# Schaudge/cellranger

Measured on AMD Instinct MI355X. Metric: M reads/sec barcode-correct+UMI-count, higher is better.
Workload: dtype u32/u64 integer keys; f64 posterior

## Files before the change

cellranger_amd/_lib.py:

```python
import ctypes as C
import os

import numpy as np

PKG = os.path.dirname(os.path.abspath(__file__))
LIB_PATH = os.environ.get("CRGPU_LIB_PATH") or os.path.join(PKG, "libcrgpu.so")

MISS = 0xFFFFFFFF
NO_FEATURE = 0xFFFFFFFF
MAX_LIB = 16
FLAG_LIB_MASK = 0x0F
FLAG_CB_HAS_N = 0x10
FLAG_NONTXOMIC = 0x20

COUNTS_VALID, COUNTS_CORRECTED, COUNTS_PRIOR = 0, 1, 2
T_NAMES = ["pack", "match", "correct", "keys", "sort_scatter", "dedup", "matrix", "synth", "sort_hist", "scan", "comm", "feature"]
UNIQUE_ID_BYTES = 128
OPT_BUFFERS_UNCHANGED_BETWEEN_CALLS = 0
STAT_SORT_REFINISHED = 1
STAT_RL_COUNTS_FROM_FINISH = 15


class CrgpuError(RuntimeError):
    def __init__(self, code, msg):
        super().__init__("crgpu error %d: %s" % (code, msg))
        self.code = code


class Records(C.Structure):
    _fields_ = [
        ("n", C.c_uint64),
        ("umi_len", C.c_uint32),
        ("d_bc_idx", C.c_void_p),
        ("d_umi", C.c_void_p),
        ("d_umi_qualn", C.c_void_p),
        ("d_feature", C.c_void_p),
        ("d_flags", C.c_void_p),
        ("d_umi_len", C.c_void_p),
        ("d_probe_idx", C.c_void_p),
    ]


class MatrixView(C.Structure):
# ... 330 lines not shown
```

cellranger_amd/csrc/common.h:

```cpp
#pragma once

#include <hip/hip_runtime.h>

#include <cstdarg>
#include <cstdint>
#include <cstdio>
#include <cstring>
#include <map>
#include <mutex>
#include <set>
#include <string>
#include <vector>

#include "../../include/crgpu.h"

#define CR_WAVE 64
#define CR_SCALAR_N_WITHOUT_FLAGS 40

struct WlTables {
    bool set = false;
    uint32_t n = 0;
    uint32_t bitsA = 0;
    uint32_t bitsB = 0;
    uint32_t *d_offA = nullptr;
// ... 115 lines not shown

    bool canon_set = false;
    uint32_t n_canon = 0, cb_len = 0;
    std::vector<uint32_t> canon_sorted;
    std::vector<uint32_t> canon_order;

    uint32_t n_segments = 0;
    uint32_t seg_n[CRGPU_MAX_SEGMENTS] = {0}, seg_len[CRGPU_MAX_SEGMENTS] = {0};
    std::vector<uint32_t> seg_seq[CRGPU_MAX_SEGMENTS];

    WlTables wl[CRGPU_MAX_LIB];
    FeaturePattern pat[CRGPU_MAX_LIB];
    FeatureExtractorSet fx[CRGPU_MAX_LIB];
    FxPendingSet fxp;
    uint32_t *d_canon_keys = nullptr;
    unsigned long long *d_hot_image = nullptr;
#define CR_REC_SETS 4
    MissRecords recs[CR_REC_SETS];
    uint32_t rec_next = 0;
    KeyHistograms ghist;
    std::map<const void *, size_t> lds_attr_done;
    uint32_t n_xcc = 0;
    uint64_t last_distinct_keys = 0, last_low_support_candidates = 0;
    uint64_t rl_counts_from_finish = 0;
    uint64_t sort_refinished = 0;
    uint64_t k1_split_rounds = 0;
    uint64_t feature_resumed_reads = 0;
    uint64_t feature_fast_launches = 0;
    uint64_t feature_reads_requeued = 0;
    uint64_t comm_bytes[3] = {0, 0, 0};
    uint64_t sort_fallbacks = 0;
    uint64_t probe_segments[3] = {0, 0, 0};
    uint32_t probe_seg_cap = 0xFFFFFFFFu;
    uint32_t ordmag_batch = 0;
    uint32_t ed_lds_features = 0xFFFFFFFFu;
    uint32_t ss_wave_min = 64, ss_wg_min = 4096, ss_task_batch = 0;

    double max_expected_errors = 1.7976931348623157e308;
    double confidence_threshold = 0.975;
    double *d_ptab = nullptr;

    KeyLayout layout;
    DenseIndex dense;
    uint8_t *d_on_target = nullptr;
    uint32_t n_target_features = 0;
    uint64_t target_min_reads = 0;
// ... 136 lines not shown
```

cellranger_amd/csrc/ctx.hip:

```cpp
#include <cmath>

#include <cstdio>
#include <cstdlib>

#include "common.h"

static thread_local std::string g_thread_err;

void cr_set_thread_error(const char *msg) { g_thread_err = msg; }

int cr_fail(crgpu_ctx *ctx, int code, const char *fmt, ...) {
    char buf[1024];
    va_list ap;
    va_start(ap, fmt);
    vsnprintf(buf, sizeof(buf), fmt, ap);
    va_end(ap);
    if (ctx)
        ctx->err = buf;
    else
        g_thread_err = buf;
    return code;
}

extern "C" int crgpu_abi_version(void) { return CRGPU_ABI_VERSION; }
// ... 246 lines not shown
        case CRGPU_STAT_COMM_BYTES_C1:
        case CRGPU_STAT_COMM_BYTES_C2:
        case CRGPU_STAT_COMM_BYTES_C3:
            *value_out = ctx->comm_bytes[which - CRGPU_STAT_COMM_BYTES_C1];
            return CRGPU_OK;
        case CRGPU_STAT_FEATURE_RESUMED_READS:
            *value_out = ctx->feature_resumed_reads;
            return CRGPU_OK;
        case CRGPU_STAT_FEATURE_FAST_LAUNCHES:
            *value_out = ctx->feature_fast_launches;
            return CRGPU_OK;
        case CRGPU_STAT_MISS_RECORD_SETS: {
            uint64_t k = 0;
            for (const MissRecords &r : ctx->recs) k += r.valid ? 1u : 0u;
            *value_out = k;
            return CRGPU_OK;
        }
        case CRGPU_STAT_DISTINCT_KEYS:
            *value_out = ctx->last_distinct_keys;
            return CRGPU_OK;
        case CRGPU_STAT_LOW_SUPPORT_CANDIDATES:
            *value_out = ctx->last_low_support_candidates;
            return CRGPU_OK;
        case CRGPU_STAT_FEATURE_READS_REQUEUED:
            *value_out = ctx->feature_reads_requeued;
            return CRGPU_OK;
        case CRGPU_STAT_PROBE_SEGMENTS_WAVE:
        case CRGPU_STAT_PROBE_SEGMENTS_WORKGROUP:
        case CRGPU_STAT_PROBE_SEGMENTS_GLOBAL:
            *value_out = ctx->probe_segments[which - CRGPU_STAT_PROBE_SEGMENTS_WAVE];
            return CRGPU_OK;
        default:
            return cr_fail(ctx, CRGPU_EINVAL, "crgpu_get_stat: unknown counter %d", which);
    }
}

void cr_invalidate(crgpu_ctx *ctx) {
    cr_drop_miss_records(ctx);
    cr_drop_feature_pending(ctx);
    ctx->ghist.valid = false;
}
void cr_invalidate_range(crgpu_ctx *ctx, const void *p, uint64_t bytes) {
    if (!p || !bytes) return;
    const uintptr_t a = (uintptr_t)p, b = a + bytes;
    auto hits = [&](const void *q, uint64_t len) { return q && (uintptr_t)q < b && (uintptr_t)q + len > a; };
    for (MissRecords &r : ctx->recs)
// ... 302 lines not shown
```

cellranger_amd/csrc/dedup.hip:

```cpp
#include "block_utils.h"
#include "common.h"

int cr_scan_small(crgpu_ctx *ctx, uint32_t *d_data, uint64_t n, uint32_t *d_total_out);
int cr_partition_by_owner(crgpu_ctx *ctx, const uint64_t *d_in, uint64_t *d_out, uint64_t n, uint32_t sh_bc,
                          uint32_t n_ranks, const uint32_t *bounds, uint64_t *counts_out);

#define NONE32 0xFFFFFFFFu

struct crgpu_counts {
    uint64_t n_triplets = 0, n_molecules = 0;
    uint32_t *d_bc = nullptr, *d_feature = nullptr, *d_count = nullptr;
    uint64_t *d_mkeys = nullptr;
    uint32_t *d_mreads = nullptr;
    uint32_t *d_corr_reads = nullptr;
    uint32_t *d_filt_reads = nullptr;
    int32_t *d_mprobe = nullptr;
    uint32_t *d_back = nullptr;
    uint32_t n_back = 0;
    uint32_t n_canon = 0;
    KeyLayout layout;
    bool pt_valid = false;
    uint32_t pt_n_probes = 0;
    uint64_t n_pt = 0;
    uint32_t *d_pt_bc = nullptr, *d_pt_probe = nullptr, *d_pt_count = nullptr;
// ... 1621 lines not shown
            rl_heads.valid = false;
        }
    }
    const uint64_t *keys = keys_rw;
    const uint32_t *vals = vals_rw;
    uint32_t nd32 = 0;
    {
        CrTimer t(ctx, CRGPU_T_DEDUP, n_keys);
        CR_TRY(run_lengths(ctx, keys, 1u, n_keys, ukey, upos, d_block, d_total, rl_heads.valid));
    }
    CR_TRY(read_u32(ctx, d_total, &nd32));
    const uint64_t nd = nd32;

    const uint64_t st_bytes = ((nd + 1) & ~1ull) * sizeof(uint16_t) + 4;
    DevBuf corr_b, incall_b, st_b, minidx_b;
    CR_TRY(dmalloc(ctx, minidx_b, nd * sizeof(uint32_t)));
    CR_TRY(dmalloc(ctx, corr_b, nd * sizeof(uint32_t)));
    CR_TRY(dmalloc(ctx, incall_b, nd * sizeof(uint32_t)));
    CR_TRY(dmalloc(ctx, st_b, st_bytes));
    uint32_t *corr = corr_b.as<uint32_t>(), *inc_all = incall_b.as<uint32_t>(), *minidx = minidx_b.as<uint32_t>();
    uint16_t *st = st_b.as<uint16_t>();
    const bool overlap = CrFork::enabled(ctx, nd);
    CrFork fork(ctx);
    DevBuf heads_b, giant_b, best_b;
    if (overlap) CR_TRY(fork.mark());
    {
        const bool timing_was = ctx->timing;
        if (overlap) ctx->timing = false;
        struct TimingBack {
            crgpu_ctx *c;
            bool v;
            ~TimingBack() { c->timing = v; }
        } timing_back{ctx, timing_was};
        CrTimer t(ctx, CRGPU_T_DEDUP);
        CR_HIP(ctx, hipMemsetAsync(inc_all, 0, nd * sizeof(uint32_t), ctx->stream));
        CR_HIP(ctx, hipMemsetAsync(st, 0, st_bytes, ctx->stream));
        CR_HIP(ctx, hipMemsetAsync(minidx, 0xFF, nd * sizeof(uint32_t), ctx->stream));
        const uint64_t n_tiles = (nd + UC_TILE - 1) / UC_TILE;
        CR_TRY(dmalloc(ctx, heads_b, 2 * n_tiles * sizeof(uint32_t)));
        uint32_t *tile_first = heads_b.as<uint32_t>(), *tile_last = tile_first + n_tiles;
#ifndef UC_GRID_WG
#define UC_GRID_WG 5u
#endif
        hipLaunchKernelGGL(k_correct_umis_tiled, dim3(cr_grid(n_tiles, 1, 256u * UC_GRID_WG)), dim3(256), 0, ctx->stream, kl, ukey,
                           upos, nd, n_keys, tile_first, tile_last, corr, st, inc_all, minidx);
        if (n_tiles > 1) {
            const size_t lds_small = (2 * UES_CAP + UES_BUCKETS * 8) * sizeof(uint32_t);
            const size_t lds_large = (2 * UE_CAP + UE_BUCKETS * 8) * sizeof(uint32_t);
            cr_allow_lds(ctx, (const void *)k_correct_umis_edges<false>, lds_large);
            cr_allow_lds(ctx, (const void *)k_giant_probe, lds_large);
            const uint64_t max_items = nd / (UE_CAP / 2) + 16;
            CR_TRY(dmalloc(ctx, giant_b, max_items * sizeof(GiantItem) + 16));
            CR_TRY(dmalloc(ctx, best_b, nd * sizeof(unsigned long long)));
            uint32_t *n_giant = reinterpret_cast<uint32_t *>(giant_b.as<unsigned char>());
            GiantItem *items = reinterpret_cast<GiantItem *>(giant_b.as<unsigned char>() + 16);
            unsigned long long *best = best_b.as<unsigned long long>();
            CR_HIP(ctx, hipMemsetAsync(n_giant, 0, sizeof(uint32_t), ctx->stream));
            hipLaunchKernelGGL(k_correct_umis_edges<true>, dim3(cr_grid(n_tiles - 1, 1, 256u * 6u)), dim3(UES_THREADS), lds_small,
                               ctx->stream, kl, ukey, upos, nd, n_keys, tile_first, tile_last, corr, st, inc_all, minidx, items, n_giant);
            hipLaunchKernelGGL(k_correct_umis_edges<false>, dim3(cr_grid(n_tiles - 1, 1, 256u * 2u)), dim3(UE_THREADS),
                               lds_large, ctx->stream, kl, ukey, upos, nd, n_keys, tile_first, tile_last, corr, st, inc_all,
                               minidx, items, n_giant);
            hipLaunchKernelGGL(k_giant_init, dim3(512), dim3(UE_THREADS), 0, ctx->stream, kl, ukey, upos, nd, n_keys, items,
                               n_giant, best);
            hipLaunchKernelGGL(k_giant_probe, dim3(512), dim3(UE_THREADS), lds_large, ctx->stream, kl, ukey, upos, nd, n_keys,
                               items, n_giant, best);
            hipLaunchKernelGGL(k_giant_final, dim3(512), dim3(UE_THREADS), 0, ctx->stream, upos, nd, n_keys, items, n_giant, best,
                               corr, st, inc_all, minidx);
        }
        CR_HIP(ctx, hipGetLastError());
    }

    {
        DevBuf cand_b, h_b, v_b;
        CR_TRY(dmalloc(ctx, cand_b, nd));
        CR_TRY(dmalloc(ctx, h_b, nd * sizeof(uint32_t)));
        CR_TRY(dmalloc(ctx, v_b, nd * sizeof(uint32_t)));
        const uint32_t vbits = cr_ceil_log2(nd ? nd : 1);
        uint32_t n_cand32 = 0;
        if (overlap) CR_TRY(fork.side(fork.t0));
        {
            CrTimer t(ctx, CRGPU_T_DEDUP);
            const uint64_t n_ftiles = (nd + LF_TILE - 1) / LF_TILE;
            hipLaunchKernelGGL(k_group_candidates, dim3(cr_grid(n_ftiles, 1, 256u * 2u)), dim3(LF_THREADS), 0, ctx->stream, kl, ukey, nd,
                               cand_b.as<uint8_t>());
// ... 92 lines not shown
        uint64_t tile;
        const uint32_t nb = cp_blocks(nd, &tile);
        const MolFlagTargeted flag_t{st, ukey, upos, inc_all, n_keys, nd, tf};
        const MolFlag flag_p{st};
        if (tf.min_reads)
            hipLaunchKernelGGL(k_mt_count<MolFlagTargeted>, dim3(nb), dim3(CP_BLOCK), 0, ctx->stream, flag_t, ukey, L.sh_feat(), nd,
                               tile, d_block, d_heads);
        else
            hipLaunchKernelGGL(k_mt_count<MolFlag>, dim3(nb), dim3(CP_BLOCK), 0, ctx->stream, flag_p, ukey, L.sh_feat(), nd, tile,
                               d_block, d_heads);
        CR_TRY(cr_scan_small(ctx, d_block, nb, d_total));
        CR_TRY(cr_scan_small(ctx, d_heads, nb, d_total_h));
        if (tf.min_reads)
            hipLaunchKernelGGL(k_mt_write<MolFlagTargeted>, dim3(nb), dim3(CP_BLOCK), 0, ctx->stream, flag_t, emit, L.sh_bc(),
                               L.sh_feat(), L.bits_feat, nd, tile, d_block, d_heads, res->d_bc, res->d_feature, tpos_b.as<uint32_t>(),
                               res->d_back);
        else
            hipLaunchKernelGGL(k_mt_write<MolFlag>, dim3(nb), dim3(CP_BLOCK), 0, ctx->stream, flag_p, emit, L.sh_bc(), L.sh_feat(),
                               L.bits_feat, nd, tile, d_block, d_heads, res->d_bc, res->d_feature, tpos_b.as<uint32_t>(), res->d_back);
        CR_HIP(ctx, hipGetLastError());
    }
    CR_TRY(read_u32(ctx, d_total, &nm32));
    CR_TRY(read_u32(ctx, d_total_h, &nt32));
    const uint64_t nm = nm32;

    if (pr.summary) {
        const size_t bytes = ((size_t)1 << L.bits_lib) * ctx->n_canon * sizeof(uint32_t);
        CR_TRY(cr_pool_alloc(ctx, (void **)&res->d_corr_reads, bytes));
        CrTimer t(ctx, CRGPU_T_DEDUP);
        CR_HIP(ctx, hipMemsetAsync(res->d_corr_reads, 0, bytes, ctx->stream));
        hipLaunchKernelGGL(k_corrected_reads, dim3(cr_grid(nd, 256)), dim3(256), 0, ctx->stream, kl, ukey, upos, nd, n_keys, st,
                           ctx->n_canon, res->d_corr_reads, res->d_back);
        if (tf.min_reads) {
            CR_TRY(cr_pool_alloc(ctx, (void **)&res->d_filt_reads, bytes));
            CR_HIP(ctx, hipMemsetAsync(res->d_filt_reads, 0, bytes, ctx->stream));
            hipLaunchKernelGGL(k_filtered_reads, dim3(cr_grid(nd, 256)), dim3(256), 0, ctx->stream, kl, ukey, upos, nd, n_keys, st,
                               inc_all, tf, ctx->n_canon, res->d_filt_reads, res->d_back);
        }
        CR_HIP(ctx, hipGetLastError());
    }

    const uint64_t nt = nt32;
    CR_TRY(cr_pool_alloc(ctx, (void **)&res->d_count, nt * sizeof(uint32_t)));
    if (nt) {
        CrTimer t(ctx, CRGPU_T_DEDUP);
        hipLaunchKernelGGL(k_trip_counts, dim3(cr_grid(nt, 256)), dim3(256), 0, ctx->stream, tpos_b.as<uint32_t>(), nt, nm, res->d_count);
// ... 827 lines not shown
```

cellranger_amd/csrc/umi_correct.h:

```cpp
#pragma once

#ifndef UC_ITEMS
#define UC_ITEMS 4
#endif
#define UC_TILE (256 * UC_ITEMS)
#ifndef UC_MIN_WG
#define UC_MIN_WG 1
#endif
#define UC_BLOCKS (UC_TILE / 64)
#ifndef UC_SMALL
#define UC_SMALL 32
#endif
#define UC_OPEN 0xFFFFu
#ifndef UC_BUCKETS
#define UC_BUCKETS 512u
#endif
#define UC_POSBITS 11u
#define UC_EMPTY 0xFFFFFFFFu
#define UC_NOCORR 0x80000000u

#define UE_THREADS 512
#define UE_CAP 4096u
#define UE_BUCKETS 1024u
#define UE_POSBITS 12u
#define UES_THREADS 256
#define UES_CAP 1024u
#define UES_BUCKETS 512u
#define UES_POSBITS 10u
#define UC_NOHEAD 0xFFFFFFFFu

struct GiantItem {
    uint32_t s, e, c0;
};

template <bool SMALL>
struct EdgeCfg;
template <>
struct EdgeCfg<true> {
    static constexpr uint32_t THREADS = UES_THREADS, CAP = UES_CAP, BUCKETS = UES_BUCKETS, POSBITS = UES_POSBITS;
};
template <>
struct EdgeCfg<false> {
    static constexpr uint32_t THREADS = UE_THREADS, CAP = UE_CAP, BUCKETS = UE_BUCKETS, POSBITS = UE_POSBITS;
};

__device__ __forceinline__ bool hd1(uint32_t a, uint32_t b) {
    const uint32_t x = a ^ b;
    const uint32_t y = (x | (x >> 1)) & 0x55555555u;
    return y != 0u && (y & (y - 1u)) == 0u;
}

struct UmiSplit {
    uint32_t lo_bits, lo_mask;
// ... 67 lines not shown
        return best.pos;
    }
    const uint32_t my_hi = my_umi >> sp.lo_bits, my_lo = my_umi & sp.lo_mask;
    for (uint32_t q = self; q > s;) {
        --q;
        const uint32_t u = s_umi[q];
        if ((u >> sp.lo_bits) != my_hi) break;
        if (hd1(u & sp.lo_mask, my_lo)) best.offer(s_cnt[q] & ~UC_NOCORR, u, q);
    }
    for (uint32_t q = self + 1; q < e; q++) {
        const uint32_t u = s_umi[q];
        if ((u >> sp.lo_bits) != my_hi) break;
        if (hd1(u & sp.lo_mask, my_lo)) best.offer(s_cnt[q] & ~UC_NOCORR, u, q);
    }
    uc_for_each<BUCKETS, POSBITS>(s_hash, seg_tag, my_lo, [&](uint32_t q) {
        const uint32_t u = s_umi[q];
        if ((u & sp.lo_mask) != my_lo) return;
        if (s_tag != nullptr && s_tag[q] != (uint16_t)seg_tag) return;
        if (hd1(u >> sp.lo_bits, my_hi)) best.offer(s_cnt[q] & ~UC_NOCORR, u, q);
    });
    return best.pos;
}

__global__ __launch_bounds__(256, UC_MIN_WG) void k_correct_umis_tiled(const KL kl, const uint64_t *__restrict__ ukey,
                                                            const uint32_t *__restrict__ upos, uint64_t nd,
                                                            uint64_t n_keys, uint32_t *__restrict__ tile_first,
                                                            uint32_t *__restrict__ tile_last, uint32_t *__restrict__ corr,
                                                            uint16_t *__restrict__ st, uint32_t *__restrict__ inc_all,
                                                            uint32_t *__restrict__ minidx) {
    __shared__ uint32_t s_umi[UC_TILE];
    __shared__ uint32_t s_cnt[UC_TILE];
    __shared__ uint16_t s_start[UC_TILE];
    __shared__ __attribute__((aligned(16))) uint32_t s_hash[UC_BUCKETS * 8];
    __shared__ unsigned long long s_heads[UC_BLOCKS];
    __shared__ int s_carry_start[UC_BLOCKS];
    __shared__ int s_carry_end[UC_BLOCKS];
    __shared__ uint32_t s_halo_head;
    __shared__ uint32_t s_any_long;
    const uint32_t tid = threadIdx.x, lane = tid & 63u;
    const uint64_t umi_mask = lowmask(kl.bits_umi);
    const UmiSplit sp = umi_split(kl.umi_len);
    const uint64_t n_tiles = (nd + UC_TILE - 1) / UC_TILE;
    for (uint32_t h = tid; h < UC_BUCKETS * 8; h += 256) s_hash[h] = UC_EMPTY;
    if (tid == 0) s_any_long = 0;
    for (uint64_t tile = blockIdx.x; tile < n_tiles; tile += gridDim.x) {
        const uint64_t t0 = tile * UC_TILE;
        const uint32_t tn = nd - t0 < UC_TILE ? (uint32_t)(nd - t0) : UC_TILE;
#pragma unroll
        for (int r = 0; r < UC_ITEMS; r++) {
            const uint32_t p = (uint32_t)r * 256u + tid;
            bool head = false;
            if (p < tn) {
                const uint64_t key = ukey[t0 + p];
                const uint64_t pre = key >> kl.sh_lib;
                head = (t0 + p == 0) || (ukey[t0 + p - 1] >> kl.sh_lib) != pre;
                s_umi[p] = (uint32_t)((key >> kl.sh_umi) & umi_mask);
                const uint32_t end = t0 + p + 1 < nd ? upos[t0 + p + 1] : (uint32_t)n_keys;
                const uint32_t lib = (uint32_t)((pre >> kl.bits_ulen) & lowmask(kl.bits_lib));
                s_cnt[p] = (end - upos[t0 + p]) | (((kl.mux_mask >> lib) & 1u) ? UC_NOCORR : 0u);
            } else {
                head = p == tn;
            }
            const unsigned long long m = __ballot(head);
            if (lane == 0) s_heads[p >> 6] = m;
        }
        if (tid == 0) {
            bool hh = true;
            if (t0 + UC_TILE < nd) hh = (ukey[t0 + UC_TILE] >> kl.sh_lib) != (ukey[t0 + UC_TILE - 1] >> kl.sh_lib);
            s_halo_head = hh ? 1u : 0u;
        }
        __syncthreads();
        if (tid < 64) {
            static_assert(UC_BLOCKS <= 64, "one lane per block");
            const unsigned long long m = tid < UC_BLOCKS ? s_heads[tid] : 0ull;
            const int last = m ? (int)(tid * 64u + 63u - (uint32_t)__clzll((long long)m)) : -1;
            const int first = m ? (int)(tid * 64u + (uint32_t)__ffsll((long long)m) - 1u) : 0x7FFFFFFF;
            int pm = last, sm = first;
#pragma unroll
            for (int d = 1; d < UC_BLOCKS; d <<= 1) {
                const int y = __shfl_up(pm, d), z = __shfl_down(sm, d);
                if ((int)tid >= d) pm = pm > y ? pm : y;
                if ((int)tid + d < (int)UC_BLOCKS) sm = sm < z ? sm : z;
            }
            int cs = __shfl_up(pm, 1), ce = __shfl_down(sm, 1);
            if (tid == 0) cs = -1;
            const int behind = s_halo_head ? (int)UC_TILE : 0x7FFFFFFF;
            if (tid + 1 >= UC_BLOCKS) ce = 0x7FFFFFFF;
            ce = ce < behind ? ce : behind;
            if (tid < UC_BLOCKS) {
                s_carry_start[tid] = cs;
                s_carry_end[tid] = ce;
            }
            unsigned long long mk = m;
            if (tid * 64u >= tn) mk = 0ull;
            else if (tn - tid * 64u < 64u) mk &= (1ull << (tn - tid * 64u)) - 1ull;
            uint32_t tf = mk ? tid * 64u + (uint32_t)__ffsll((long long)mk) - 1u : UC_NOHEAD;
            int tl = mk ? (int)(tid * 64u + 63u - (uint32_t)__clzll((long long)mk)) : -1;
#pragma unroll
            for (int d = 32; d >= 1; d >>= 1) {
                const uint32_t y = __shfl_xor(tf, d);
                const int z = __shfl_xor(tl, d);
                tf = tf < y ? tf : y;
                tl = tl > z ? tl : z;
            }
            if (tid == 0) {
                tile_first[tile] = tf;
                tile_last[tile] = tl >= 0 ? (uint32_t)tl : UC_NOHEAD;
            }
        }
        __syncthreads();
        bool inserted = false;
#pragma unroll
        for (int r = 0; r < UC_ITEMS; r++) {
            const uint32_t p = (uint32_t)r * 256u + tid;
            if (p >= tn) continue;
            const uint32_t b = p >> 6;
            const unsigned long long heads = s_heads[b];
            const unsigned long long le = heads & ((2ull << lane) - 1ull);
            const int start = le ? (int)(b * 64u + 63u - (uint32_t)__clzll((long long)le)) : s_carry_start[b];
            const unsigned long long gt = lane < 63u ? (heads >> (lane + 1u)) : 0ull;
            const int end = gt ? (int)(p + (uint32_t)__ffsll((long long)gt)) : s_carry_end[b];
            const bool closed = start >= 0 && end <= (int)UC_TILE;
            s_start[p] = closed ? (uint16_t)start : (uint16_t)UC_OPEN;
            if (closed && end - start > UC_SMALL && !(s_cnt[p] & UC_NOCORR)) {
                uc_insert<UC_BUCKETS, UC_POSBITS>(s_hash, (uint32_t)start, s_umi[p] & sp.lo_mask, p);
                inserted = true;
            }
        }
        if (inserted) s_any_long = 1;
        __syncthreads();
#pragma unroll 1
        for (int r = 0; r < UC_ITEMS; r++) {
            const uint32_t p = (uint32_t)r * 256u + tid;
            if (p >= tn) continue;
            const uint32_t s = s_start[p];
            if (s == UC_OPEN) continue;
            const uint32_t eb = p >> 6;
            const unsigned long long gt = lane < 63u ? (s_heads[eb] >> (lane + 1u)) : 0ull;
            const uint32_t e = gt ? p + (uint32_t)__ffsll((long long)gt) : (uint32_t)s_carry_end[eb];
            const uint64_t k = t0 + p;
            const uint32_t cw = s_cnt[p];
            const uint32_t my_cnt = cw & ~UC_NOCORR;
            uint32_t target = NONE32;
            if (!(cw & UC_NOCORR) && e - s > 1) {
                const uint32_t bp = best_neighbour_lds<UC_BUCKETS, UC_POSBITS>(s_umi, s_cnt, s_hash, s_start, s, e, s, p,
                                                                              s_umi[p], my_cnt, sp);
                if (bp != p) target = (uint32_t)(t0 + bp);
            }
            if (target != NONE32) move_reads(corr, st, inc_all, minidx, k, target, my_cnt);
        }
        __syncthreads();
        if (s_any_long) {
            for (uint32_t h = tid; h < UC_BUCKETS * 8; h += 256) s_hash[h] = UC_EMPTY;
            __syncthreads();
            if (tid == 0) s_any_long = 0;
        }
    }
}

template <bool SMALL>
__global__ __launch_bounds__(EdgeCfg<SMALL>::THREADS) void k_correct_umis_edges(
    const KL kl, const uint64_t *__restrict__ ukey, const uint32_t *__restrict__ upos, uint64_t nd, uint64_t n_keys,
    const uint32_t *__restrict__ tile_first, const uint32_t *__restrict__ tile_last, uint32_t *__restrict__ corr,
    uint16_t *__restrict__ st, uint32_t *__restrict__ inc_all, uint32_t *__restrict__ minidx, GiantItem *__restrict__ giant_items,
    uint32_t *__restrict__ n_giant) {
    constexpr uint32_t UE_T = EdgeCfg<SMALL>::THREADS, CAP = EdgeCfg<SMALL>::CAP, BUCKETS = EdgeCfg<SMALL>::BUCKETS,
                       POSBITS = EdgeCfg<SMALL>::POSBITS;
    extern __shared__ __attribute__((aligned(16))) uint32_t smem[];
    uint32_t *s_umi = smem;
    uint32_t *s_cnt = smem + CAP;
    uint32_t *s_hash = smem + 2 * CAP;
    const uint32_t tid = threadIdx.x;
    const uint64_t umi_mask = lowmask(kl.bits_umi);
    const UmiSplit sp = umi_split(kl.umi_len);
    const uint64_t n_tiles = (nd + UC_TILE - 1) / UC_TILE;
    for (uint64_t t = (uint64_t)blockIdx.x + 1; t < n_tiles; t += gridDim.x) {
        const uint32_t tf = tile_first[t];
        if (tf == 0u) continue;
        const uint32_t tl = tile_last[t - 1];
        if (tl == UC_NOHEAD) continue;
        const uint64_t s = (t - 1) * UC_TILE + tl;
        uint64_t e = nd;
        if (tf != UC_NOHEAD) {
            e = t * UC_TILE + tf;
        } else {
            for (uint64_t u = t + 1; u < n_tiles; u++) {
                const uint32_t f = tile_first[u];
                if (f != UC_NOHEAD) {
                    e = u * UC_TILE + f;
                    break;
                }
            }
        }
        const uint64_t m = e - s;
        if (SMALL ? m > UES_CAP : m <= UES_CAP) continue;
        const uint32_t lib = (uint32_t)((ukey[s] >> kl.sh_libid) & lowmask(kl.bits_lib));
        if ((kl.mux_mask >> lib) & 1u) continue;
        if (m <= CAP) {
            const uint32_t mm = (uint32_t)m;
            const bool use_hash = mm > UC_SMALL;
            if (use_hash)
                for (uint32_t h = tid; h < BUCKETS * 8; h += UE_T) s_hash[h] = UC_EMPTY;
            for (uint32_t p = tid; p < mm; p += UE_T) {
                const uint64_t k = s + p;
                s_umi[p] = (uint32_t)((ukey[k] >> kl.sh_umi) & umi_mask);
                s_cnt[p] = run_count(upos, nd, n_keys, k);
            }
            __syncthreads();
            if (use_hash) {
                for (uint32_t p = tid; p < mm; p += UE_T)
                    uc_insert<BUCKETS, POSBITS>(s_hash, 0u, s_umi[p] & sp.lo_mask, p);
                __syncthreads();
            }
            for (uint32_t p = tid; p < mm; p += UE_T) {
                const uint32_t my_cnt = s_cnt[p];
                const uint32_t bp = best_neighbour_lds<BUCKETS, POSBITS>(s_umi, s_cnt, s_hash, nullptr, 0u, mm, 0u, p,
                                                                              s_umi[p], my_cnt, sp);
                if (bp != p) move_reads(corr, st, inc_all, minidx, s + p, (uint32_t)(s + bp), my_cnt);
            }
            __syncthreads();
            continue;
        }
        {
            __shared__ uint32_t s_item0;
            const uint32_t n_chunks = (uint32_t)((m + CAP - 1) / CAP);
            if (tid == 0) s_item0 = atomicAdd(n_giant, n_chunks);
            __syncthreads();
            const uint32_t item0 = s_item0;
            for (uint32_t c = tid; c < n_chunks; c += UE_T)
                giant_items[item0 + c] = GiantItem{(uint32_t)s, (uint32_t)e, (uint32_t)(s + (uint64_t)c * CAP)};
            __syncthreads();
        }
    }
}

#define GI_HALO 512u
__global__ __launch_bounds__(UE_THREADS) void k_giant_init(const KL kl, const uint64_t *__restrict__ ukey,
                                                           const uint32_t *__restrict__ upos, uint64_t nd, uint64_t n_keys,
                                                           const GiantItem *__restrict__ items,
                                                           const uint32_t *__restrict__ n_items_ptr,
                                                           unsigned long long *__restrict__ best) {
    __shared__ uint32_t s_u[UE_CAP + 2 * GI_HALO], s_c[UE_CAP + 2 * GI_HALO];
    const uint32_t n_items = *n_items_ptr;
    const uint64_t umi_mask = lowmask(kl.bits_umi);
    const UmiSplit sp = umi_split(kl.umi_len);
    for (uint32_t it = blockIdx.x; it < n_items; it += gridDim.x) {
        const GiantItem g = items[it];
        const uint64_t s = g.s, e = g.e;
        const uint64_t c1 = (uint64_t)g.c0 + UE_CAP < e ? (uint64_t)g.c0 + UE_CAP : e;
        const uint64_t w0 = (uint64_t)g.c0 >= s + GI_HALO ? (uint64_t)g.c0 - GI_HALO : s;
        const uint64_t w1 = c1 + GI_HALO < e ? c1 + GI_HALO : e;
        __syncthreads();
        for (uint64_t k = w0 + threadIdx.x; k < w1; k += UE_THREADS) {
            s_u[k - w0] = (uint32_t)((ukey[k] >> kl.sh_umi) & umi_mask);
            s_c[k - w0] = run_count(upos, nd, n_keys, k);
// ... 116 lines not shown
```

include/crgpu.h:

```cpp
#ifndef CRGPU_H
#define CRGPU_H

#include <stddef.h>
#include <stdint.h>

#ifdef __cplusplus
extern "C" {
#endif

#define CRGPU_ABI_VERSION 3
#define CRGPU_MAX_LIB 16
#define CRGPU_MISS 0xFFFFFFFFu
#define CRGPU_NO_FEATURE 0xFFFFFFFFu

#define CRGPU_OK 0
#define CRGPU_EINVAL (-1)
#define CRGPU_ENODEV (-2)
#define CRGPU_EHIP (-3)
#define CRGPU_ENOMEM (-4)
#define CRGPU_ESTATE (-5)
#define CRGPU_ERANGE (-6)
#define CRGPU_ECOMM (-7)

#define CRGPU_FLAG_LIB_MASK 0x0Fu
// ... 9 lines not shown
int crgpu_local_group_id(uint32_t n_ranks, void *id_out);
int crgpu_create(crgpu_ctx **out, int device_id, int n_ranks, int rank, const void *unique_id);
void crgpu_destroy(crgpu_ctx *ctx);
int crgpu_comm_info(crgpu_ctx *ctx, uint32_t *n_ranks_out, uint32_t *rank_out);
#define CRGPU_OPT_BUFFERS_UNCHANGED_BETWEEN_CALLS 0
#define CRGPU_OPT_DENSE_BARCODE_KEYS 1
int crgpu_set_option(crgpu_ctx *ctx, int option, int64_t value);
int crgpu_invalidate(crgpu_ctx *ctx);
#define CRGPU_STAT_SORT_FALLBACKS 0
#define CRGPU_STAT_K1_SPLIT_ROUNDS 3
#define CRGPU_STAT_FEATURE_READS_REQUEUED 2
#define CRGPU_STAT_FEATURE_FAST_LAUNCHES 4
#define CRGPU_STAT_FEATURE_RESUMED_READS 8
#define CRGPU_STAT_COMM_BYTES_C1 5
#define CRGPU_STAT_COMM_BYTES_C2 6
#define CRGPU_STAT_COMM_BYTES_C3 7
#define CRGPU_STAT_DISTINCT_KEYS 9
#define CRGPU_STAT_LOW_SUPPORT_CANDIDATES 10
#define CRGPU_STAT_MISS_RECORD_SETS 11
#define CRGPU_STAT_SORT_REFINISHED 1
#define CRGPU_STAT_PROBE_SEGMENTS_WAVE 12
#define CRGPU_STAT_PROBE_SEGMENTS_WORKGROUP 13
#define CRGPU_STAT_PROBE_SEGMENTS_GLOBAL 14
#define CRGPU_STAT_RL_COUNTS_FROM_FINISH 15
int crgpu_get_stat(crgpu_ctx *ctx, int which, uint64_t *value_out);
const char *crgpu_last_error(const crgpu_ctx *ctx);
int crgpu_synchronize(crgpu_ctx *ctx);
void *crgpu_stream(crgpu_ctx *ctx);
int crgpu_malloc(crgpu_ctx *ctx, void **d_out, uint64_t bytes);
int crgpu_free(crgpu_ctx *ctx, void *d_ptr);
int crgpu_trim(crgpu_ctx *ctx);
int crgpu_memcpy_h2d(crgpu_ctx *ctx, void *d_dst, const void *h_src, uint64_t bytes);
int crgpu_memcpy_d2h(crgpu_ctx *ctx, void *h_dst, const void *d_src, uint64_t bytes);
int crgpu_memset(crgpu_ctx *ctx, void *d_dst, int value, uint64_t bytes);

#define CRGPU_T_PACK 0
#define CRGPU_T_MATCH 1
#define CRGPU_T_CORRECT 2
#define CRGPU_T_KEYS 3
#define CRGPU_T_SORT 4
#define CRGPU_T_DEDUP 5
#define CRGPU_T_MATRIX 6
#define CRGPU_T_SYNTH 7
#define CRGPU_T_SORT_HIST 8
#define CRGPU_T_SCAN 9
#define CRGPU_T_COMM 10
// ... 467 lines not shown
```

Before: 17190.

## Correct UMIs per wavefront window with halo and queue long segments for edge kernels

Replaces the 256-thread tiled UMI-correction kernel with a kernel where each wavefront owns a 256-key window plus a halo of up to 256 keys. Each wave keeps its own LDS tables and syncs only at wave level instead of with block barriers. Segments that run past the halo are located with a ballot scan plus galloping search and appended to a compact long-segment queue, split by size. The edge kernels now read that queue instead of scanning per-tile head arrays, and they prefetch the next item's keys into registers. This adds a device-to-host readback for a new stat counter and extra LDS per block, which may lower occupancy.

```diff
diff --git a/cellranger_amd/_lib.py b/cellranger_amd/_lib.py
--- a/cellranger_amd/_lib.py
+++ b/cellranger_amd/_lib.py
@@ -19,6 +19,7 @@
 OPT_BUFFERS_UNCHANGED_BETWEEN_CALLS = 0
 STAT_SORT_REFINISHED = 1
 STAT_RL_COUNTS_FROM_FINISH = 15
+STAT_LONG_SEGMENTS = 16
 
 
 class CrgpuError(RuntimeError):
diff --git a/cellranger_amd/csrc/common.h b/cellranger_amd/csrc/common.h
--- a/cellranger_amd/csrc/common.h
+++ b/cellranger_amd/csrc/common.h
@@ -161,6 +161,7 @@
     std::map<const void *, size_t> lds_attr_done;
     uint32_t n_xcc = 0;
     uint64_t last_distinct_keys = 0, last_low_support_candidates = 0;
+    uint64_t last_long_segments = 0;
     uint64_t rl_counts_from_finish = 0;
     uint64_t sort_refinished = 0;
     uint64_t k1_split_rounds = 0;
diff --git a/cellranger_amd/csrc/ctx.hip b/cellranger_amd/csrc/ctx.hip
--- a/cellranger_amd/csrc/ctx.hip
+++ b/cellranger_amd/csrc/ctx.hip
@@ -292,6 +292,9 @@
         case CRGPU_STAT_LOW_SUPPORT_CANDIDATES:
             *value_out = ctx->last_low_support_candidates;
             return CRGPU_OK;
+        case CRGPU_STAT_LONG_SEGMENTS:
+            *value_out = ctx->last_long_segments;
+            return CRGPU_OK;
         case CRGPU_STAT_FEATURE_READS_REQUEUED:
             *value_out = ctx->feature_reads_requeued;
             return CRGPU_OK;
diff --git a/cellranger_amd/csrc/dedup.hip b/cellranger_amd/csrc/dedup.hip
--- a/cellranger_amd/csrc/dedup.hip
+++ b/cellranger_amd/csrc/dedup.hip
@@ -1667,7 +1667,8 @@
     uint16_t *st = st_b.as<uint16_t>();
     const bool overlap = CrFork::enabled(ctx, nd);
     CrFork fork(ctx);
-    DevBuf heads_b, giant_b, best_b;
+    DevBuf long_b, giant_b, best_b;
+    uint32_t *n_long = ctx->d_scalars + 18;
     if (overlap) CR_TRY(fork.mark());
     {
         const bool timing_was = ctx->timing;
@@ -1681,15 +1682,14 @@
         CR_HIP(ctx, hipMemsetAsync(inc_all, 0, nd * sizeof(uint32_t), ctx->stream));
         CR_HIP(ctx, hipMemsetAsync(st, 0, st_bytes, ctx->stream));
         CR_HIP(ctx, hipMemsetAsync(minidx, 0xFF, nd * sizeof(uint32_t), ctx->stream));
-        const uint64_t n_tiles = (nd + UC_TILE - 1) / UC_TILE;
-        CR_TRY(dmalloc(ctx, heads_b, 2 * n_tiles * sizeof(uint32_t)));
-        uint32_t *tile_first = heads_b.as<uint32_t>(), *tile_last = tile_first + n_tiles;
-#ifndef UC_GRID_WG
-#define UC_GRID_WG 5u
-#endif
-        hipLaunchKernelGGL(k_correct_umis_tiled, dim3(cr_grid(n_tiles, 1, 256u * UC_GRID_WG)), dim3(256), 0, ctx->stream, kl, ukey,
-                           upos, nd, n_keys, tile_first, tile_last, corr, st, inc_all, minidx);
-        if (n_tiles > 1) {
+        const uint64_t n_win = (nd + UCW_W - 1) / UCW_W;
+        const uint32_t max_long = (uint32_t)(nd / UCW_H + 16);
+        CR_TRY(dmalloc(ctx, long_b, (uint64_t)max_long * sizeof(LongSeg)));
+        LongSeg *long_items = long_b.as<LongSeg>();
+        CR_HIP(ctx, hipMemsetAsync(n_long, 0, 2 * sizeof(uint32_t), ctx->stream));
+        hipLaunchKernelGGL(k_correct_umis_waves, dim3(cr_grid(n_win, UCW_WAVES, 256u * UCW_GRID_WG)), dim3(64u * UCW_WAVES), 0,
+                           ctx->stream, kl, ukey, upos, nd, n_keys, corr, st, inc_all, minidx, long_items, n_long, max_long);
+        if (nd > UCW_H) {
             const size_t lds_small = (2 * UES_CAP + UES_BUCKETS * 8) * sizeof(uint32_t);
             const size_t lds_large = (2 * UE_CAP + UE_BUCKETS * 8) * sizeof(uint32_t);
             cr_allow_lds(ctx, (const void *)k_correct_umis_edges<false>, lds_large);
@@ -1701,11 +1701,12 @@
             GiantItem *items = reinterpret_cast<GiantItem *>(giant_b.as<unsigned char>() + 16);
             unsigned long long *best = best_b.as<unsigned long long>();
             CR_HIP(ctx, hipMemsetAsync(n_giant, 0, sizeof(uint32_t), ctx->stream));
-            hipLaunchKernelGGL(k_correct_umis_edges<true>, dim3(cr_grid(n_tiles - 1, 1, 256u * 6u)), dim3(UES_THREADS), lds_small,
-                               ctx->stream, kl, ukey, upos, nd, n_keys, tile_first, tile_last, corr, st, inc_all, minidx, items, n_giant);
-            hipLaunchKernelGGL(k_correct_umis_edges<false>, dim3(cr_grid(n_tiles - 1, 1, 256u * 2u)), dim3(UE_THREADS),
-                               lds_large, ctx->stream, kl, ukey, upos, nd, n_keys, tile_first, tile_last, corr, st, inc_all,
-                               minidx, items, n_giant);
+            hipLaunchKernelGGL(k_correct_umis_edges<true>, dim3(cr_grid(max_long, 1, 256u * 6u)), dim3(UES_THREADS), lds_small,
+                               ctx->stream, kl, ukey, upos, nd, n_keys, long_items, n_long, max_long, corr, st, inc_all, minidx, items,
+                               n_giant);
+            hipLaunchKernelGGL(k_correct_umis_edges<false>, dim3(cr_grid(max_long, 1, 256u * 2u)), dim3(UE_THREADS), lds_large,
+                               ctx->stream, kl, ukey, upos, nd, n_keys, long_items, n_long, max_long, corr, st, inc_all, minidx, items,
+                               n_giant);
             hipLaunchKernelGGL(k_giant_init, dim3(512), dim3(UE_THREADS), 0, ctx->stream, kl, ukey, upos, nd, n_keys, items,
                                n_giant, best);
             hipLaunchKernelGGL(k_giant_probe, dim3(512), dim3(UE_THREADS), lds_large, ctx->stream, kl, ukey, upos, nd, n_keys,
@@ -1844,6 +1845,11 @@
     }
     CR_TRY(read_u32(ctx, d_total, &nm32));
     CR_TRY(read_u32(ctx, d_total_h, &nt32));
+    {
+        uint32_t nl[2] = {0, 0};
+        CR_TRY(crgpu_memcpy_d2h(ctx, nl, n_long, sizeof(nl)));
+        ctx->last_long_segments = (uint64_t)nl[0] + nl[1];
+    }
     const uint64_t nm = nm32;
 
     if (pr.summary) {
diff --git a/cellranger_amd/csrc/umi_correct.h b/cellranger_amd/csrc/umi_correct.h
--- a/cellranger_amd/csrc/umi_correct.h
+++ b/cellranger_amd/csrc/umi_correct.h
@@ -1,21 +1,30 @@
 #pragma once
 
-#ifndef UC_ITEMS
-#define UC_ITEMS 4
+#ifndef UCW_W
+#define UCW_W 256u
 #endif
-#define UC_TILE (256 * UC_ITEMS)
-#ifndef UC_MIN_WG
-#define UC_MIN_WG 1
+#ifndef UCW_H
+#define UCW_H 256u
 #endif
-#define UC_BLOCKS (UC_TILE / 64)
+#ifndef UCW_WAVES
+#define UCW_WAVES 4u
+#endif
+#ifndef UCW_GRID_WG
+#define UCW_GRID_WG 4u
+#endif
+#ifndef UCW_BUCKETS
+#define UCW_BUCKETS 128u
+#endif
+#define UCW_T (UCW_W + UCW_H)
+#define UCW_WB (UCW_W / 64u)
+#define UCW_NB (UCW_T / 64u)
+#define UCW_POSBITS 9u
+static_assert(UCW_W % 64u == 0 && UCW_H % 64u == 0 && UCW_W >= 64u && UCW_H >= 64u, "whole blocks of 64 keys");
+static_assert(UCW_T <= (1u << UCW_POSBITS) && UCW_T <= UCW_BUCKETS * 8u, "positions fit a slot, entries fit the table");
 #ifndef UC_SMALL
 #define UC_SMALL 32
 #endif
 #define UC_OPEN 0xFFFFu
-#ifndef UC_BUCKETS
-#define UC_BUCKETS 512u
-#endif
-#define UC_POSBITS 11u
 #define UC_EMPTY 0xFFFFFFFFu
 #define UC_NOCORR 0x80000000u
 
@@ -27,8 +36,10 @@
 #define UES_CAP 1024u
 #define UES_BUCKETS 512u
 #define UES_POSBITS 10u
-#define UC_NOHEAD 0xFFFFFFFFu
-
+
+struct LongSeg {
+    uint32_t s, e;
+};
 struct GiantItem {
     uint32_t s, e, c0;
 };
@@ -142,138 +153,175 @@
     return best.pos;
 }
 
-__global__ __launch_bounds__(256, UC_MIN_WG) void k_correct_umis_tiled(const KL kl, const uint64_t *__restrict__ ukey,
-                                                            const uint32_t *__restrict__ upos, uint64_t nd,
-                                                            uint64_t n_keys, uint32_t *__restrict__ tile_first,
-                                                            uint32_t *__restrict__ tile_last, uint32_t *__restrict__ corr,
-                                                            uint16_t *__restrict__ st, uint32_t *__restrict__ inc_all,
-                                                            uint32_t *__restrict__ minidx) {
-    __shared__ uint32_t s_umi[UC_TILE];
-    __shared__ uint32_t s_cnt[UC_TILE];
-    __shared__ uint16_t s_start[UC_TILE];
-    __shared__ __attribute__((aligned(16))) uint32_t s_hash[UC_BUCKETS * 8];
-    __shared__ unsigned long long s_heads[UC_BLOCKS];
-    __shared__ int s_carry_start[UC_BLOCKS];
-    __shared__ int s_carry_end[UC_BLOCKS];
-    __shared__ uint32_t s_halo_head;
-    __shared__ uint32_t s_any_long;
-    const uint32_t tid = threadIdx.x, lane = tid & 63u;
+__device__ __forceinline__ void uc_wave_sync() {
+    __builtin_amdgcn_fence(__ATOMIC_RELEASE, "wavefront");
+    __builtin_amdgcn_wave_barrier();
+    __builtin_amdgcn_fence(__ATOMIC_ACQUIRE, "wavefront");
+}
+
+__device__ __forceinline__ uint64_t uc_find_end(const uint64_t *__restrict__ ukey, uint64_t nd, uint64_t from, uint64_t pre,
+                                                uint32_t shift, uint32_t lane) {
+    for (uint32_t r = 0; r < 4u; r++) {
+        const uint64_t b = from + r * 256u;
+        uint64_t k[4];
+#pragma unroll
+        for (uint32_t j = 0; j < 4u; j++) {
+            const uint64_t g = b + j * 64u + lane;
+            k[j] = ukey[g < nd ? g : nd - 1];
+        }
+#pragma unroll
+        for (uint32_t j = 0; j < 4u; j++) {
+            const uint64_t g = b + j * 64u + lane;
+            const unsigned long long m = __ballot(g >= nd || (k[j] >> shift) != pre);
+            if (m) return b + j * 64u + (uint32_t)__ffsll((long long)m) - 1u;
+        }
+    }
+    uint64_t lo = from + 1023u, step = 1024u;
+    while (lo + step < nd && (ukey[lo + step] >> shift) == pre) {
+        lo += step;
+        step <<= 1;
+    }
+    uint64_t a = lo, b = lo + step < nd ? lo + step - 1 : nd - 1;
+    while (a < b) {
+        const uint64_t mid = (a + b + 1) >> 1;
+        if ((ukey[mid] >> shift) == pre) a = mid; else b = mid - 1;
+    }
+    return a + 1;
+}
+
+__global__ __launch_bounds__(64 * UCW_WAVES) void k_correct_umis_waves(const KL kl, const uint64_t *__restrict__ ukey,
+                                                                      const uint32_t *__restrict__ upos, uint64_t nd,
+                                                                      uint64_t n_keys, uint32_t *__restrict__ corr,
+                                                                      uint16_t *__restrict__ st, uint32_t *__restrict__ inc_all,
+                                                                      uint32_t *__restrict__ minidx, LongSeg *__restrict__ long_items,
+                                                                      uint32_t *__restrict__ n_long, uint32_t max_long) {
+    __shared__ uint32_t s_umi_w[UCW_WAVES][UCW_T];
+    __shared__ uint32_t s_cnt_w[UCW_WAVES][UCW_T];
+    __shared__ uint16_t s_start_w[UCW_WAVES][UCW_T];
+    __shared__ __attribute__((aligned(16))) uint32_t s_hash_w[UCW_WAVES][UCW_BUCKETS * 8];
+    __shared__ unsigned long long s_heads_w[UCW_WAVES][UCW_NB];
+    __shared__ int s_ce_w[UCW_WAVES][UCW_NB];
+    const uint32_t lane = threadIdx.x & 63u, wv = threadIdx.x >> 6;
+    uint32_t *s_umi = s_umi_w[wv], *s_cnt = s_cnt_w[wv], *s_hash = s_hash_w[wv];
+    uint16_t *s_start = s_start_w[wv];
+    unsigned long long *s_heads = s_heads_w[wv];
+    int *s_ce = s_ce_w[wv];
     const uint64_t umi_mask = lowmask(kl.bits_umi);
     const UmiSplit sp = umi_split(kl.umi_len);
-    const uint64_t n_tiles = (nd + UC_TILE - 1) / UC_TILE;
-    for (uint32_t h = tid; h < UC_BUCKETS * 8; h += 256) s_hash[h] = UC_EMPTY;
-    if (tid == 0) s_any_long = 0;
-    for (uint64_t tile = blockIdx.x; tile < n_tiles; tile += gridDim.x) {
-        const uint64_t t0 = tile * UC_TILE;
-        const uint32_t tn = nd - t0 < UC_TILE ? (uint32_t)(nd - t0) : UC_TILE;
-#pragma unroll
-        for (int r = 0; r < UC_ITEMS; r++) {
-            const uint32_t p = (uint32_t)r * 256u + tid;
-            bool head = false;
-            if (p < tn) {
-                const uint64_t key = ukey[t0 + p];
-                const uint64_t pre = key >> kl.sh_lib;
-                head = (t0 + p == 0) || (ukey[t0 + p - 1] >> kl.sh_lib) != pre;
-                s_umi[p] = (uint32_t)((key >> kl.sh_umi) & umi_mask);
-                const uint32_t end = t0 + p + 1 < nd ? upos[t0 + p + 1] : (uint32_t)n_keys;
-                const uint32_t lib = (uint32_t)((pre >> kl.bits_ulen) & lowmask(kl.bits_lib));
-                s_cnt[p] = (end - upos[t0 + p]) | (((kl.mux_mask >> lib) & 1u) ? UC_NOCORR : 0u);
-            } else {
-                head = p == tn;
-            }
+    const uint64_t n_win = (nd + UCW_W - 1) / UCW_W;
+    const uint4 empty4 = make_uint4(UC_EMPTY, UC_EMPTY, UC_EMPTY, UC_EMPTY);
+    for (uint32_t h = lane; h < UCW_BUCKETS * 2u; h += 64u) reinterpret_cast<uint4 *>(s_hash)[h] = empty4;
+    uc_wave_sync();
+    for (uint64_t win = (uint64_t)blockIdx.x * UCW_WAVES + wv; win < n_win; win += (uint64_t)gridDim.x * UCW_WAVES) {
+        const uint64_t w0 = win * UCW_W;
+        auto stage = [&](uint32_t j) -> unsigned long long {
+            const uint32_t p = j * 64u + lane;
+            const uint64_t g = w0 + p;
+            const bool valid = g < nd;
+            const uint64_t gc = valid ? g : nd - 1;
+            const uint64_t key = ukey[gc];
+            const uint64_t prev = ukey[gc ? gc - 1 : 0];
+            const uint32_t up0 = upos[gc];
+            const uint32_t up1 = upos[gc + 1 < nd ? gc + 1 : gc];
+            const uint64_t pre = key >> kl.sh_lib;
+            const bool head = !valid || g == 0 || (prev >> kl.sh_lib) != pre;
+            const uint32_t end = gc + 1 < nd ? up1 : (uint32_t)n_keys;
+            const uint32_t lib = (uint32_t)((pre >> kl.bits_ulen) & lowmask(kl.bits_lib));
+            s_umi[p] = (uint32_t)((key >> kl.sh_umi) & umi_mask);
+            s_cnt[p] = (end - up0) | (((kl.mux_mask >> lib) & 1u) ? UC_NOCORR : 0u);
             const unsigned long long m = __ballot(head);
-            if (lane == 0) s_heads[p >> 6] = m;
-        }
-        if (tid == 0) {
-            bool hh = true;
-            if (t0 + UC_TILE < nd) hh = (ukey[t0 + UC_TILE] >> kl.sh_lib) != (ukey[t0 + UC_TILE - 1] >> kl.sh_lib);
-            s_halo_head = hh ? 1u : 0u;
-        }
-        __syncthreads();
-        if (tid < 64) {
-            static_assert(UC_BLOCKS <= 64, "one lane per block");
-            const unsigned long long m = tid < UC_BLOCKS ? s_heads[tid] : 0ull;
-            const int last = m ? (int)(tid * 64u + 63u - (uint32_t)__clzll((long long)m)) : -1;
-            const int first = m ? (int)(tid * 64u + (uint32_t)__ffsll((long long)m) - 1u) : 0x7FFFFFFF;
-            int pm = last, sm = first;
-#pragma unroll
-            for (int d = 1; d < UC_BLOCKS; d <<= 1) {
-                const int y = __shfl_up(pm, d), z = __shfl_down(sm, d);
-                if ((int)tid >= d) pm = pm > y ? pm : y;
-                if ((int)tid + d < (int)UC_BLOCKS) sm = sm < z ? sm : z;
-            }
-            int cs = __shfl_up(pm, 1), ce = __shfl_down(sm, 1);
-            if (tid == 0) cs = -1;
-            const int behind = s_halo_head ? (int)UC_TILE : 0x7FFFFFFF;
-            if (tid + 1 >= UC_BLOCKS) ce = 0x7FFFFFFF;
-            ce = ce < behind ? ce : behind;
-            if (tid < UC_BLOCKS) {
-                s_carry_start[tid] = cs;
-                s_carry_end[tid] = ce;
-            }
-            unsigned long long mk = m;
-            if (tid * 64u >= tn) mk = 0ull;
-            else if (tn - tid * 64u < 64u) mk &= (1ull << (tn - tid * 64u)) - 1ull;
-            uint32_t tf = mk ? tid * 64u + (uint32_t)__ffsll((long long)mk) - 1u : UC_NOHEAD;
-            int tl = mk ? (int)(tid * 64u + 63u - (uint32_t)__clzll((long long)mk)) : -1;
-#pragma unroll
-            for (int d = 32; d >= 1; d >>= 1) {
-                const uint32_t y = __shfl_xor(tf, d);
-                const int z = __shfl_xor(tl, d);
-                tf = tf < y ? tf : y;
-                tl = tl > z ? tl : z;
-            }
-            if (tid == 0) {
-                tile_first[tile] = tf;
-                tile_last[tile] = tl >= 0 ? (uint32_t)tl : UC_NOHEAD;
-            }
-        }
-        __syncthreads();
+            if (lane == 0) s_heads[j] = m;
+            return m;
+        };
+        unsigned long long hm[UCW_NB];
+#pragma unroll
+        for (uint32_t j = 0; j <= UCW_WB; j++) hm[j] = stage(j);
+        uint32_t nblk = UCW_WB + 1u;
+        bool found = hm[UCW_WB] != 0ull;
+#pragma unroll
+        for (uint32_t j = UCW_WB + 1u; j < UCW_NB; j++) {
+            hm[j] = 0ull;
+            if (!found) {
+                hm[j] = stage(j);
+                nblk = j + 1u;
+                found = hm[j] != 0ull;
+            }
+        }
+        bool halo_head = false;
+        if (!found) {
+            const uint64_t gt = w0 + UCW_T;
+            halo_head = gt >= nd || (ukey[gt < nd ? gt : nd - 1] >> kl.sh_lib) != (ukey[gt - 1] >> kl.sh_lib);
+        }
+        int cs[UCW_NB], ce[UCW_NB];
+        {
+            int run = -1;
+#pragma unroll
+            for (uint32_t j = 0; j < UCW_NB; j++) {
+                cs[j] = run;
+                if (hm[j]) run = (int)(j * 64u + 63u - (uint32_t)__clzll((long long)hm[j]));
+            }
+            int nxt = halo_head ? (int)UCW_T : 0x7FFFFFFF;
+#pragma unroll
+            for (int j = (int)UCW_NB - 1; j >= 0; j--) {
+                ce[j] = nxt;
+                if (lane == 0) s_ce[j] = nxt;
+                if (hm[j]) nxt = (int)((uint32_t)j * 64u + (uint32_t)__ffsll((long long)hm[j]) - 1u);
+            }
+        }
         bool inserted = false;
 #pragma unroll
-        for (int r = 0; r < UC_ITEMS; r++) {
-            const uint32_t p = (uint32_t)r * 256u + tid;
-            if (p >= tn) continue;
-            const uint32_t b = p >> 6;
-            const unsigned long long heads = s_heads[b];
+        for (uint32_t j = 0; j < UCW_NB; j++) {
+            if (j >= nblk) continue;
+            const uint32_t p = j * 64u + lane;
+            const unsigned long long heads = hm[j];
             const unsigned long long le = heads & ((2ull << lane) - 1ull);
-            const int start = le ? (int)(b * 64u + 63u - (uint32_t)__clzll((long long)le)) : s_carry_start[b];
+            const int start = le ? (int)(j * 64u + 63u - (uint32_t)__clzll((long long)le)) : cs[j];
             const unsigned long long gt = lane < 63u ? (heads >> (lane + 1u)) : 0ull;
-            const int end = gt ? (int)(p + (uint32_t)__ffsll((long long)gt)) : s_carry_end[b];
-            const bool closed = start >= 0 && end <= (int)UC_TILE;
-            s_start[p] = closed ? (uint16_t)start : (uint16_t)UC_OPEN;
-            if (closed && end - start > UC_SMALL && !(s_cnt[p] & UC_NOCORR)) {
-                uc_insert<UC_BUCKETS, UC_POSBITS>(s_hash, (uint32_t)start, s_umi[p] & sp.lo_mask, p);
+            const int end = gt ? (int)(p + (uint32_t)__ffsll((long long)gt)) : ce[j];
+            const bool mine = w0 + p < nd && start >= 0 && start < (int)UCW_W && end <= (int)UCW_T;
+            s_start[p] = mine ? (uint16_t)start : (uint16_t)UC_OPEN;
+            if (mine && end - start > UC_SMALL && !(s_cnt[p] & UC_NOCORR)) {
+                uc_insert<UCW_BUCKETS, UCW_POSBITS>(s_hash, (uint32_t)start, s_umi[p] & sp.lo_mask, p);
                 inserted = true;
             }
         }
-        if (inserted) s_any_long = 1;
-        __syncthreads();
+        uc_wave_sync();
 #pragma unroll 1
-        for (int r = 0; r < UC_ITEMS; r++) {
-            const uint32_t p = (uint32_t)r * 256u + tid;
-            if (p >= tn) continue;
+        for (uint32_t j = 0; j < nblk; j++) {
+            const uint32_t p = j * 64u + lane;
             const uint32_t s = s_start[p];
             if (s == UC_OPEN) continue;
-            const uint32_t eb = p >> 6;
-            const unsigned long long gt = lane < 63u ? (s_heads[eb] >> (lane + 1u)) : 0ull;
-            const uint32_t e = gt ? p + (uint32_t)__ffsll((long long)gt) : (uint32_t)s_carry_end[eb];
-            const uint64_t k = t0 + p;
+            const unsigned long long gt = lane < 63u ? (s_heads[j] >> (lane + 1u)) : 0ull;
+            const uint32_t e = gt ? p + (uint32_t)__ffsll((long long)gt) : (uint32_t)s_ce[j];
             const uint32_t cw = s_cnt[p];
             const uint32_t my_cnt = cw & ~UC_NOCORR;
-            uint32_t target = NONE32;
             if (!(cw & UC_NOCORR) && e - s > 1) {
-                const uint32_t bp = best_neighbour_lds<UC_BUCKETS, UC_POSBITS>(s_umi, s_cnt, s_hash, s_start, s, e, s, p,
-                                                                              s_umi[p], my_cnt, sp);
-                if (bp != p) target = (uint32_t)(t0 + bp);
-            }
-            if (target != NONE32) move_reads(corr, st, inc_all, minidx, k, target, my_cnt);
-        }
-        __syncthreads();
-        if (s_any_long) {
-            for (uint32_t h = tid; h < UC_BUCKETS * 8; h += 256) s_hash[h] = UC_EMPTY;
-            __syncthreads();
-            if (tid == 0) s_any_long = 0;
+                const uint32_t bp = best_neighbour_lds<UCW_BUCKETS, UCW_POSBITS>(s_umi, s_cnt, s_hash, s_start, s, e, s, p, s_umi[p],
+                                                                                  my_cnt, sp);
+                if (bp != p) move_reads(corr, st, inc_all, minidx, w0 + p, (uint32_t)(w0 + bp), my_cnt);
+            }
+        }
+        if (cs[UCW_WB] >= 0 && ce[UCW_WB - 1u] > (int)UCW_T) {
+            const uint64_t s = w0 + (uint32_t)cs[UCW_WB];
+            const uint64_t hk = ukey[s];
+            const uint32_t lib = (uint32_t)((hk >> kl.sh_libid) & lowmask(kl.bits_lib));
+            if (!((kl.mux_mask >> lib) & 1u)) {
+                const uint64_t e = uc_find_end(ukey, nd, w0 + UCW_T, hk >> kl.sh_lib, kl.sh_lib, lane);
+                if (lane == 0) {
+                    if (e - s <= UES_CAP) {
+                        const uint32_t at = atomicAdd(&n_long[0], 1u);
+                        if (at < max_long) long_items[at] = LongSeg{(uint32_t)s, (uint32_t)e};
+                    } else {
+                        const uint32_t at = atomicAdd(&n_long[1], 1u);
+                        if (at < max_long) long_items[max_long - 1u - at] = LongSeg{(uint32_t)s, (uint32_t)e};
+                    }
+                }
+            }
+        }
+        uc_wave_sync();
+        if (__ballot(inserted)) {
+            for (uint32_t h = lane; h < UCW_BUCKETS * 2u; h += 64u) reinterpret_cast<uint4 *>(s_hash)[h] = empty4;
+            uc_wave_sync();
         }
     }
 }
@@ -281,11 +329,11 @@
 template <bool SMALL>
 __global__ __launch_bounds__(EdgeCfg<SMALL>::THREADS) void k_correct_umis_edges(
     const KL kl, const uint64_t *__restrict__ ukey, const uint32_t *__restrict__ upos, uint64_t nd, uint64_t n_keys,
-    const uint32_t *__restrict__ tile_first, const uint32_t *__restrict__ tile_last, uint32_t *__restrict__ corr,
+    const LongSeg *__restrict__ long_items, const uint32_t *__restrict__ n_long, uint32_t max_long, uint32_t *__restrict__ corr,
     uint16_t *__restrict__ st, uint32_t *__restrict__ inc_all, uint32_t *__restrict__ minidx, GiantItem *__restrict__ giant_items,
     uint32_t *__restrict__ n_giant) {
     constexpr uint32_t UE_T = EdgeCfg<SMALL>::THREADS, CAP = EdgeCfg<SMALL>::CAP, BUCKETS = EdgeCfg<SMALL>::BUCKETS,
-                       POSBITS = EdgeCfg<SMALL>::POSBITS;
+                       POSBITS = EdgeCfg<SMALL>::POSBITS, PER = CAP / UE_T;
     extern __shared__ __attribute__((aligned(16))) uint32_t smem[];
     uint32_t *s_umi = smem;
     uint32_t *s_cnt = smem + CAP;
@@ -293,40 +341,46 @@
     const uint32_t tid = threadIdx.x;
     const uint64_t umi_mask = lowmask(kl.bits_umi);
     const UmiSplit sp = umi_split(kl.umi_len);
-    const uint64_t n_tiles = (nd + UC_TILE - 1) / UC_TILE;
-    for (uint64_t t = (uint64_t)blockIdx.x + 1; t < n_tiles; t += gridDim.x) {
-        const uint32_t tf = tile_first[t];
-        if (tf == 0u) continue;
-        const uint32_t tl = tile_last[t - 1];
-        if (tl == UC_NOHEAD) continue;
-        const uint64_t s = (t - 1) * UC_TILE + tl;
-        uint64_t e = nd;
-        if (tf != UC_NOHEAD) {
-            e = t * UC_TILE + tf;
-        } else {
-            for (uint64_t u = t + 1; u < n_tiles; u++) {
-                const uint32_t f = tile_first[u];
-                if (f != UC_NOHEAD) {
-                    e = u * UC_TILE + f;
-                    break;
-                }
-            }
-        }
+    const uint32_t n_items = n_long[SMALL ? 0 : 1] < max_long ? n_long[SMALL ? 0 : 1] : max_long;
+    uint64_t rk[PER];
+    uint32_t r0[PER], r1[PER];
+    auto item_at = [&](uint32_t it) { return long_items[SMALL ? it : max_long - 1u - it]; };
+    auto request = [&](const LongSeg g) {
+        if (g.e - g.s > CAP) return;
+#pragma unroll
+        for (uint32_t i = 0; i < PER; i++) {
+            const uint64_t k = (uint64_t)g.s + i * UE_T + tid;
+            const uint64_t kc = k < g.e ? k : (uint64_t)g.e - 1;
+            rk[i] = ukey[kc];
+            r0[i] = upos[kc];
+            r1[i] = upos[kc + 1 < nd ? kc + 1 : kc];
+        }
+    };
+    uint32_t it = blockIdx.x;
+    if (it >= n_items) return;
+    LongSeg cur = item_at(it);
+    request(cur);
+    for (; it < n_items; it += gridDim.x) {
+        const bool has_next = it + gridDim.x < n_items;
+        LongSeg nxt = cur;
+        if (has_next) nxt = item_at(it + gridDim.x);
+        const uint64_t s = cur.s, e = cur.e;
         const uint64_t m = e - s;
-        if (SMALL ? m > UES_CAP : m <= UES_CAP) continue;
-        const uint32_t lib = (uint32_t)((ukey[s] >> kl.sh_libid) & lowmask(kl.bits_lib));
-        if ((kl.mux_mask >> lib) & 1u) continue;
         if (m <= CAP) {
             const uint32_t mm = (uint32_t)m;
             const bool use_hash = mm > UC_SMALL;
             if (use_hash)
                 for (uint32_t h = tid; h < BUCKETS * 8; h += UE_T) s_hash[h] = UC_EMPTY;
-            for (uint32_t p = tid; p < mm; p += UE_T) {
-                const uint64_t k = s + p;
-                s_umi[p] = (uint32_t)((ukey[k] >> kl.sh_umi) & umi_mask);
-                s_cnt[p] = run_count(upos, nd, n_keys, k);
+#pragma unroll
+            for (uint32_t i = 0; i < PER; i++) {
+                const uint32_t p = i * UE_T + tid;
+                if (p < mm) {
+                    s_umi[p] = (uint32_t)((rk[i] >> kl.sh_umi) & umi_mask);
+                    s_cnt[p] = (s + p + 1 < nd ? r1[i] : (uint32_t)n_keys) - r0[i];
+                }
             }
             __syncthreads();
+            if (has_next) request(nxt);
             if (use_hash) {
                 for (uint32_t p = tid; p < mm; p += UE_T)
                     uc_insert<BUCKETS, POSBITS>(s_hash, 0u, s_umi[p] & sp.lo_mask, p);
@@ -339,9 +393,7 @@
                 if (bp != p) move_reads(corr, st, inc_all, minidx, s + p, (uint32_t)(s + bp), my_cnt);
             }
             __syncthreads();
-            continue;
-        }
-        {
+        } else {
             __shared__ uint32_t s_item0;
             const uint32_t n_chunks = (uint32_t)((m + CAP - 1) / CAP);
             if (tid == 0) s_item0 = atomicAdd(n_giant, n_chunks);
@@ -350,7 +402,9 @@
             for (uint32_t c = tid; c < n_chunks; c += UE_T)
                 giant_items[item0 + c] = GiantItem{(uint32_t)s, (uint32_t)e, (uint32_t)(s + (uint64_t)c * CAP)};
             __syncthreads();
-        }
+            if (has_next) request(nxt);
+        }
+        cur = nxt;
     }
 }
 
diff --git a/include/crgpu.h b/include/crgpu.h
--- a/include/crgpu.h
+++ b/include/crgpu.h
@@ -55,6 +55,7 @@
 #define CRGPU_STAT_PROBE_SEGMENTS_WAVE 12
 #define CRGPU_STAT_PROBE_SEGMENTS_WORKGROUP 13
 #define CRGPU_STAT_PROBE_SEGMENTS_GLOBAL 14
+#define CRGPU_STAT_LONG_SEGMENTS 16
 #define CRGPU_STAT_RL_COUNTS_FROM_FINISH 15
 int crgpu_get_stat(crgpu_ctx *ctx, int which, uint64_t *value_out);
 const char *crgpu_last_error(const crgpu_ctx *ctx);
```

New measurement: 16890. 0.982x the previous value.
